# conix-center/pointcloud_stitching

Measured on AMD Instinct MI355X. Metric: Mpoints/s stitched (8x1280x720 streams: deproject+transform+RGB+pack), higher is better.
Workload: dtype f32

## Files before the change

pointcloud_stitching_amd/csrc/pcs_kernels.hip:

```cpp

#include "pcs_kernels_common.h"

#ifndef EMIT_WAVES
#define EMIT_WAVES 6
#endif

#ifndef PCS_SCALAR_FP64
#define PCS_SCALAR_FP64 0
#endif
#ifndef SCALAR_DENSE_WAVES
#define SCALAR_DENSE_WAVES 7
#endif
#ifndef SCALAR_EMIT_CUT_WAVES
#define SCALAR_EMIT_CUT_WAVES 5
#endif

namespace pcs {

namespace {

constexpr uint32_t kDenseStageBytes = kTilePoints * PCS_POINT_BYTES;
constexpr uint32_t kStageBytes      = kTilePoints * PCS_POINT_BYTES + 32;

__device__ __forceinline__ void stage_record(uint8_t* lds, uint32_t off, const Record& r)
// ... 73 lines not shown
#pragma unroll
            for (int k = 0; k < 8; k++) {
                const size_t i = (size_t)i0 + k;
                if (i < n) p[k] = PointIn{vertices[3 * i], vertices[3 * i + 1], vertices[3 * i + 2], texcoords[2 * i], texcoords[2 * i + 1]};
                else p[k] = PointIn{0, 0, 0, 0, 0};
            }
        }
    }
};

template <uint32_t THREADS = kBlockThreads>
__device__ __forceinline__ void store_staged(const uint8_t* lds, uint32_t head, uint32_t nbytes, uint8_t* g)
{
    uint8_t* g0 = g - head;
    const uint32_t end = head + nbytes;
    const uint32_t first_full = (head + 15u) >> 4;
    const uint32_t last_full = end >> 4;
    typedef uint32_t u32x4 __attribute__((ext_vector_type(4)));
    for (uint32_t j = first_full + threadIdx.x; j < last_full; j += THREADS)
        __builtin_nontemporal_store(reinterpret_cast<const u32x4*>(lds)[j], reinterpret_cast<u32x4*>(g0) + j);
    const uint32_t head_end = min(first_full << 4, end);
    for (uint32_t b = head + 2u * threadIdx.x; b < head_end; b += 2u * THREADS)
        *reinterpret_cast<uint16_t*>(g0 + b) = *reinterpret_cast<const uint16_t*>(lds + b);
    if (last_full >= first_full) {
        const uint32_t tail_begin = max(last_full << 4, head_end);
        for (uint32_t b = tail_begin + 2u * threadIdx.x; b < end; b += 2u * THREADS)
            *reinterpret_cast<uint16_t*>(g0 + b) = *reinterpret_cast<const uint16_t*>(lds + b);
    }
}

template <class Src, uint32_t THREADS = kBlockThreads, class Arith = SimdArith>
__device__ __forceinline__ void dense_tile(const StreamParams& P, const Src& src, const uint8_t* __restrict__ color,
                                           uint32_t tile0, uint32_t n, uint8_t* __restrict__ out_bytes,
                                           uint4* stage)
{
    const uint32_t i0 = tile0 + threadIdx.x * kPointsPerLane;
    PointIn p[8];
    src.load8(P, i0, n, p);

    uint32_t w[20];
    auto fill = [&](auto& cv) {
#pragma unroll
        for (int k = 0; k < 8; k += 2) {
            const Record a = make_record<Arith>(P, color, p[k], cv);
            const Record b = make_record<Arith>(P, color, p[k + 1], cv);
            uint32_t* o = w + (k >> 1) * 5;
            o[0] = a.xy;
            o[1] = a.zc;
            o[2] = perm(b.xy, a.b, kLoLo);
            o[3] = perm(b.zc, b.xy, kHiLo);
            o[4] = perm(b.b, b.zc, kHiLo);
        }
    };
    if (Src::Math::kCvtMode == 2) {
        FastCvt<false> fast;
        fill(fast);
        if (__builtin_expect(fast.redo(), 0)) { ExactCvt exact; fill(exact); }
    } else if (Src::Math::kCvtMode == 1) {
        FastCvt<true> fast;
        fill(fast);
        if (__builtin_expect(fast.redo(), 0)) { ExactCvt exact; fill(exact); }
    } else {
        ExactCvt exact;
        fill(exact);
    }
    uint4* mine = stage + threadIdx.x * 5;
#pragma unroll
    for (int k = 0; k < 5; k++) mine[k] = make_uint4(w[4 * k], w[4 * k + 1], w[4 * k + 2], w[4 * k + 3]);
    __syncthreads();

    const uint32_t pts = min(THREADS * kPointsPerLane, n - tile0);
    store_staged<THREADS>(reinterpret_cast<const uint8_t*>(stage), 0u, pts * PCS_POINT_BYTES,
                          out_bytes + (size_t)tile0 * PCS_POINT_BYTES);
}

constexpr uint32_t kWaveStageBytes = 64u * kPointsPerLane * PCS_POINT_BYTES;
constexpr uint32_t kWinPieces      = 3;
constexpr uint32_t kWinBytes       = kWinPieces * 64u * 16u;
constexpr uint32_t kWinZeroWord    = kWaveStageBytes - 16u;
static_assert(kWinBytes + 8u <= kWinZeroWord, "the windows, the dword read past their end and the zero word fit one wave's stage");

template <class T> using cptr = const __attribute__((address_space(4))) T*;

__device__ __forceinline__ void color_stretch(const StreamParams& P, const int32_t (&wp)[3], int32_t crow, int32_t c0, int32_t c1,
                                              uint32_t room, uint32_t& ws, uint32_t& len)
{
    const int32_t lo = min(max((c0 * wp[0] + wp[1]) >> 12, 0), P.cW - 1);
    const int32_t hi = min(max((c1 * wp[0] + wp[2]) >> 12, 0), P.cW - 1);
    const uint32_t row = (uint32_t)crow * (uint32_t)P.stride;
    ws = (row + (uint32_t)lo * (uint32_t)P.bpp) & ~15u;
    const uint32_t we = min((row + (uint32_t)hi * (uint32_t)P.bpp + 4u + 15u) & ~15u, P.color_bytes & ~15u);
    len = min(we > ws ? we - ws : 0u, room);
}

typedef uint32_t u32x4v __attribute__((ext_vector_type(4)));
__device__ __forceinline__ u32x4v load16_asm(const void* base, uint32_t off)
{
    u32x4v v;
    asm volatile("global_load_dwordx4 %0, %1, %2" : "=v"(v) : "v"(off), "s"(base));
    return v;
}
__device__ __forceinline__ uint32_t load4_asm(const void* base, uint32_t off)
{
    uint32_t v;
    asm volatile("global_load_dword %0, %1, %2" : "=v"(v) : "v"(off), "s"(base));
    return v;
}
__device__ __forceinline__ void window_piece(const uint8_t* color, uint32_t off, uint32_t lds)
{
    uint32_t keep;
    asm volatile("s_mov_b32 %0, m0\n\ts_mov_b32 m0, %3\n\ts_nop 0\n\tglobal_load_lds_dwordx4 %1, %2\n\ts_mov_b32 m0, %0"
                 : "=&s"(keep) : "v"(off), "s"(color), "s"(lds) : "memory");
}

template <class Mth>
__device__ __forceinline__ PointIn deproject_pixel_win(const StreamParams& P, uint32_t d, float mx, float my)
{
    const float z = __fmul_rn(P.depth_scale, (float)d);
    PointIn p;
    p.X = __fmul_rn(z, mx);
    p.Y = __fmul_rn(z, my);
    p.Z = z;
    const float P0 = __fadd_rn(p.X, P.t[0]);
    const float P2 = p.Z;
    float x, y_unused;
    Mth::div2(P0, P0, P2, x, y_unused);
    const float px = __fadd_rn(__fmul_rn(x, P.c_fx), P.c_ppx);
    p.u = Mth::div_const(px, P.c_w_f, P.c_rw);
    p.v = 0.0f;
    return p;
}

template <class Mth, uint32_t THREADS = kBlockThreads>
__device__ __forceinline__ void dense_tile_rowc(const StreamParams& P, const uint16_t* __restrict__ depth,
                                                const uint8_t* __restrict__ color, uint32_t tile0, uint32_t n,
                                                uint8_t* __restrict__ out_bytes, uint4* stage)
{
    static_assert(Mth::kRowConst && Mth::kCvtMode == 2, "the no-overflow row-constant policy");
    const uint32_t i0 = tile0 + threadIdx.x * kPointsPerLane;
    const uint32_t ic = min(i0, n - kPointsPerLane);
    const uint32_t r = P.w_magic ? (__umulhi(ic, P.w_magic) >> P.w_shift) : ic / (uint32_t)P.W;
    const uint32_t c0 = ic - r * (uint32_t)P.W;
    u32x4v dv = load16_asm(depth, ic * 2u);
    u32x4v ma = load16_asm(P.mx, c0 * 4u);
    u32x4v mb = load16_asm(P.mx, c0 * 4u + 16u);
    uint32_t myb = load4_asm(P.my, r * 4u);
    uint32_t crow = load4_asm(P.my, ((uint32_t)P.H + r) * 4u);

    const uint32_t wave = __builtin_amdgcn_readfirstlane(threadIdx.x >> 6);
    const uint32_t iw = tile0 + wave * 64u * kPointsPerLane;
    const uint32_t il = min(iw + 64u * kPointsPerLane, n) - 1u;
    const uint32_t ra = __builtin_amdgcn_readfirstlane(r), rb = __builtin_amdgcn_readlane(r, 63);
    const cptr<int32_t> tab = (cptr<int32_t>)(uintptr_t)(P.my + P.H);
    const int32_t wp[3] = {tab[P.H], tab[P.H + 1], tab[P.H + 2]};
    const uint32_t lrel = wave * kWaveStageBytes;
    uint32_t wsa = 0, lena = 0, wsb = 0, lenb = 0;
    if (iw < n) {
        color_stretch(P, wp, tab[ra], (int32_t)(iw - ra * (uint32_t)P.W), ra == rb ? (int32_t)(il - ra * (uint32_t)P.W) : P.W - 1,
                      kWinBytes, wsa, lena);
        if (rb != ra) color_stretch(P, wp, tab[rb], 0, (int32_t)(il - rb * (uint32_t)P.W), kWinBytes - lena, wsb, lenb);
    }
    const uint32_t lane = threadIdx.x & 63u;
    const uint32_t pieces = max((lena + lenb) >> 4, 1u), pa = lena >> 4;
    const uint32_t lds0 = (uint32_t)(uintptr_t)(__attribute__((address_space(3))) uint8_t*)stage + lrel;
#pragma unroll
    for (uint32_t k = 0; k < kWinPieces; k++) {
        const uint32_t j = min(k * 64u + lane, pieces - 1u);
        window_piece(color, j < pa ? wsa + 16u * j : wsb + 16u * (j - pa), lds0 + k * 1024u);
    }
    if (lane == 0) *reinterpret_cast<uint32_t*>(reinterpret_cast<uint8_t*>(stage) + lrel + kWinZeroWord) = *(cptr<uint32_t>)(uintptr_t)color;
    float M[12];
#pragma unroll
    for (int k = 0; k < 12; k++) M[k] = P.M[k];
    float c_wm1_f = P.c_wm1_f;
    uint32_t bpp = (uint32_t)P.bpp, stride = (uint32_t)P.stride;
    asm volatile("" : "+s"(M[0]), "+s"(M[1]), "+s"(M[2]), "+s"(M[3]), "+s"(M[4]), "+s"(M[5]), "+s"(M[6]), "+s"(M[7]), "+s"(M[8]),
                      "+s"(M[9]), "+s"(M[10]), "+s"(M[11]), "+s"(c_wm1_f), "+s"(bpp), "+s"(stride));
    static_assert(kWinPieces == 3, "the wait below leaves the window's requests in flight");
    asm volatile("s_waitcnt vmcnt(3)" : "+v"(dv), "+v"(ma), "+v"(mb), "+v"(myb), "+v"(crow));
    PointIn p[8];
    {
        const uint32_t dw[4] = {dv.x, dv.y, dv.z, dv.w};
        const uint32_t mxs[8] = {ma.x, ma.y, ma.z, ma.w, mb.x, mb.y, mb.z, mb.w};
#pragma unroll
        for (int k = 0; k < 8; k++) {
            const uint32_t d = (k & 1) ? (dw[k >> 1] >> 16) : (dw[k >> 1] & 0xFFFFu);
            p[k] = deproject_pixel_win<Mth>(P, d, __uint_as_float(mxs[k]), __uint_as_float(myb));
        }
    }
    FastCvt<false> cv;
    uint32_t xy[8], zz[8], ci[8];
    const uint32_t row_off = __umul24(crow, stride);
#pragma unroll
    for (int k = 0; k < 8; k++) {
        const float ax = world_mm(M + 0, p[k].X, p[k].Y, p[k].Z);
        const float ay = world_mm(M + 4, p[k].X, p[k].Y, p[k].Z);
        const float az = world_mm(M + 8, p[k].X, p[k].Y, p[k].Z);
        xy[k] = perm((uint32_t)cv.cvt(ay), (uint32_t)cv.cvt(ax), kLoLo);
        zz[k] = (uint32_t)cv.cvt(az);
        const int32_t xi = cv.pixel(__fmaf_rn(p[k].u, P.c_w_f, 0.5f), P.cW - 1, c_wm1_f);
        ci[k] = p[k].Z != 0.0f ? __umul24((uint32_t)xi, bpp) + row_off : 0u;
    }
    const bool in_a = r == ra;
    const uint32_t ws = in_a ? wsa : wsb, len = in_a ? lena : lenb;
    const uint32_t wn = len > 3u ? len - 3u : 0u;
    const uint32_t lb = lrel + (in_a ? 0u : lena), lz = lrel + kWinZeroWord;
    asm volatile("s_waitcnt vmcnt(0)" : "+v"(ci[0]), "+v"(ci[1]), "+v"(ci[2]), "+v"(ci[3]), "+v"(ci[4]), "+v"(ci[5]), "+v"(ci[6]),
                 "+v"(ci[7]) :: "memory");
    uint32_t wc[8];
    bool miss = false;
#pragma unroll
    for (int k = 0; k < 8; k++) {
        const uint32_t o = ci[k] - ws;
        const bool in = o < wn;
        const uint32_t* qa = reinterpret_cast<const uint32_t*>(reinterpret_cast<const uint8_t*>(stage) + (in ? (lb + o) & ~3u : lz));
        wc[k] = __builtin_amdgcn_alignbyte(qa[1], qa[0], ci[k]);
        miss |= !in && ci[k] != 0u;
    }
    if (__builtin_expect(miss, 0)) {
#pragma unroll
        for (int k = 0; k < 8; k++) {
            if (!(ci[k] - ws < wn) && ci[k] != 0u) {
                ExactCvt exact;
                uint32_t shift;
                const uint32_t off = exact.window(ci[k], P.color_bytes - 4u, shift);
                uint32_t g;
                __builtin_memcpy(&g, color + off, 4);
                wc[k] = g >> shift;
            }
        }
    }
    uint32_t w[20];
#pragma unroll
    for (int k = 0; k < 8; k += 2) {
        const Record a{xy[k], perm(wc[k], zz[k], kLoLo), __builtin_amdgcn_ubfe(wc[k], 16, 8)};
        const Record b{xy[k + 1], perm(wc[k + 1], zz[k + 1], kLoLo), __builtin_amdgcn_ubfe(wc[k + 1], 16, 8)};
        uint32_t* o = w + (k >> 1) * 5;
        o[0] = a.xy;
        o[1] = a.zc;
        o[2] = perm(b.xy, a.b, kLoLo);
        o[3] = perm(b.zc, b.xy, kHiLo);
        o[4] = perm(b.b, b.zc, kHiLo);
    }
    uint4* mine = stage + threadIdx.x * 5;
#pragma unroll
    for (int k = 0; k < 5; k++) mine[k] = make_uint4(w[4 * k], w[4 * k + 1], w[4 * k + 2], w[4 * k + 3]);
    __syncthreads();

    const uint32_t pts = min(THREADS * kPointsPerLane, n - tile0);
    store_staged<THREADS>(reinterpret_cast<const uint8_t*>(stage), 0u, pts * PCS_POINT_BYTES,
                          out_bytes + (size_t)tile0 * PCS_POINT_BYTES);
}

template <class Src, bool PRED, bool DS1, class Arith = SimdArith>
__device__ __forceinline__ void generic_tile(const StreamParams& P, const Src& src, const uint8_t* __restrict__ color,
                                             uint32_t tile0, uint32_t n, uint32_t flags, uint32_t ds,
                                             uint32_t g0, uint32_t out_first, uint8_t* __restrict__ payload_bytes,
                                             uint8_t* stage, uint32_t* wsum)
{
    if (DS1) ds = 1u;
    const uint32_t i0 = tile0 + threadIdx.x * kPointsPerLane;
    PointIn p[8];
    src.load8(P, i0, n, p);

    uint32_t keep, ex = 0;
    if (PRED) {
        keep = keep_mask8(p, i0, n, flags);
        uint32_t wave_total;
        ex = wave_exclusive_scan(__popc(keep), wave_total);
        if ((threadIdx.x & 63) == 63) wsum[threadIdx.x >> 6] = wave_total;
    } else {
        const uint32_t mine = (i0 < n) ? min(8u, n - i0) : 0u;
        keep = (1u << mine) - 1u;
    }

    Record rec[8];
    auto fill = [&](auto& cv) {
#pragma unroll
        for (int k = 0; k < 8; k++) rec[k] = make_record<Arith>(P, color, p[k], cv);
    };
    if (Src::Math::kCvtMode == 2) {
        FastCvt<false> fast;
        fill(fast);
        if (__builtin_expect(fast.redo(), 0)) { ExactCvt exact; fill(exact); }
    } else if (Src::Math::kCvtMode == 1) {
        FastCvt<true> fast;
        fill(fast);
        if (__builtin_expect(fast.redo(), 0)) { ExactCvt exact; fill(exact); }
    } else {
        ExactCvt exact;
        fill(exact);
    }

    uint32_t lane_first, tile_kept;
    if (PRED) {
        __syncthreads();
        const int wave = threadIdx.x >> 6;
        uint32_t before = 0;
        for (int w = 0; w < wave; w++) before += wsum[w];
        tile_kept = wsum[0] + wsum[1] + wsum[2] + wsum[3];
        lane_first = before + ex;
    } else {
        const uint32_t pts = min(kTilePoints, n - tile0);
        lane_first = min(threadIdx.x * kPointsPerLane, pts);
        tile_kept = pts;
    }

    const uint32_t q_lo = out_first + (DS1 ? g0 : (g0 + ds - 1) / ds);
    const uint32_t q_hi = out_first + (DS1 ? g0 + tile_kept : (g0 + tile_kept + ds - 1) / ds);
    uint8_t* gdst = payload_bytes + (size_t)q_lo * PCS_POINT_BYTES;
    const uint32_t head = (uint32_t)((uintptr_t)gdst & 15u);

    uint32_t g = g0 + lane_first;
// ... 76 lines not shown
    const uint32_t n = P.n_points;
    const uint32_t tile0 = t * kTilePoints;
    const uint32_t i0 = tile0 + threadIdx.x * kPointsPerLane;
    const uint8_t* __restrict__ color = fp.color[s];

    DepthSource<true, true, Mth> src{fp.depth[s]};
    PointIn p[8];
    src.load8(P, i0, n, p);
    const uint32_t keep = keep_mask8(p, i0, n, a.flags);

    uint32_t wave_total;
    const uint32_t ex = wave_exclusive_scan(__popc(keep), wave_total);
    const int wave = threadIdx.x >> 6, lane = threadIdx.x & 63;
    if (lane == 63) wsum[wave] = wave_total;
    __syncthreads();
    uint32_t before = 0;
    for (int w = 0; w < wave; w++) before += wsum[w];
    const uint32_t tile_kept = wsum[0] + wsum[1] + wsum[2] + wsum[3];
    const uint32_t lane_first = before + ex;

    if (threadIdx.x == 0)
        __hip_atomic_store(a.desc + gtile, desc_pack(a.gen, kDescReady, tile_kept), __ATOMIC_RELAXED,
                           __HIP_MEMORY_SCOPE_AGENT);

    Record rec[8];
    auto fill = [&](auto& cv) {
#pragma unroll
        for (int k = 0; k < 8; k++) rec[k] = make_record(P, color, p[k], cv);
    };
    if (Mth::kCvtMode == 2) {
        FastCvt<false> fast;
        fill(fast);
        if (__builtin_expect(fast.redo(), 0)) { ExactCvt exact; fill(exact); }
    } else if (Mth::kCvtMode == 1) {
        FastCvt<true> fast;
        fill(fast);
        if (__builtin_expect(fast.redo(), 0)) { ExactCvt exact; fill(exact); }
    } else {
        ExactCvt exact;
        fill(exact);
    }

    uint32_t own = 0, tot = 0;
    const uint32_t first = gtile - t;
    for (uint32_t j = first + threadIdx.x; j < gtile; j += kBlockThreads) own += desc_wait(a.desc + j, a.gen, a.error);
    if ((int)threadIdx.x < s) tot = desc_wait(a.stream_desc + stream0 + threadIdx.x, a.gen, a.error);
    const uint32_t tot_lane = tot;
    own = wave_sum(own);
    tot = wave_sum(tot);
    if (lane == 0) { psum[wave] = own; psum[4 + wave] = tot; }
    __syncthreads();
    const uint32_t own_excl = psum[0] + psum[1] + psum[2] + psum[3];
    const uint32_t chain = a.chain_in ? *a.chain_in : 0u;
    const uint32_t q_lo = chain + psum[4] + psum[5] + psum[6] + psum[7] + own_excl;
    if (threadIdx.x == 0 && t == tiles_s - 1) {
        __hip_atomic_store(a.stream_desc + stream0 + s, desc_pack(a.gen, kDescReady, own_excl + tile_kept), __ATOMIC_RELAXED,
                           __HIP_MEMORY_SCOPE_AGENT);
        a.stream_end[stream0 + s] = q_lo + tile_kept;
    }
    if (a.counts && s == n_launch - 1 && t == tiles_s - 1) {
        if ((int)threadIdx.x < s) a.counts[stream0 + threadIdx.x] = (int32_t)tot_lane;
        if (threadIdx.x == 0) {
            a.counts[stream0 + s] = (int32_t)(own_excl + tile_kept);
            if (a.last_launch) a.counts[a.n_total] = (int32_t)(q_lo + tile_kept);
        }
    }

    uint8_t* gdst = payload_bytes + (size_t)q_lo * PCS_POINT_BYTES;
    const uint32_t head = (uint32_t)((uintptr_t)gdst & 15u);
    uint32_t rank = lane_first;
#pragma unroll
    for (int k = 0; k < 8; k++) {
        if ((keep >> k) & 1u) {
            stage_record(stage, head + rank * PCS_POINT_BYTES, rec[k]);
            rank++;
        }
    }
    __syncthreads();
    store_staged(stage, head, tile_kept * PCS_POINT_BYTES, gdst);
}



template <bool DDIST, bool CDIST, class Mth, uint32_t THREADS = kBlockThreads>
__global__ __launch_bounds__(THREADS, 7)
void pcs_fused_dense_kernel(const StreamParams* __restrict__ params, int stream0, FramePtrs fp,
                            uint8_t* __restrict__ payload_bytes)
{
    __shared__ uint4 stage[THREADS * kPointsPerLane * PCS_POINT_BYTES / 16];
    const int s = blockIdx.y;
    const StreamParams& P = params[stream0 + s];
    request_constants(P, fp.depth[s], fp.color[s], payload_bytes);
    const uint32_t n = P.n_points;
    const uint32_t tile0 = blockIdx.x * (THREADS * kPointsPerLane);
    if (tile0 >= n) return;
    if constexpr (Mth::kRowConst) {
        dense_tile_rowc<Mth, THREADS>(P, fp.depth[s], fp.color[s], tile0, n, payload_bytes + (size_t)P.out_base * PCS_POINT_BYTES, stage);
    } else {
        DepthSource<DDIST, CDIST, Mth> src{fp.depth[s]};
        dense_tile<DepthSource<DDIST, CDIST, Mth>, THREADS>(P, src, fp.color[s], tile0, n, payload_bytes + (size_t)P.out_base * PCS_POINT_BYTES, stage);
    }
}

template <bool DDIST, bool CDIST, class Mth>
__global__ __launch_bounds__(kBlockThreads, 7)
void pcs_fused_dense_batch_kernel(const StreamParams* __restrict__ params, BatchPtrs bp)
{
    __shared__ uint4 stage[kDenseStageBytes / 16];
    const int s = blockIdx.y;
    const StreamParams& P = params[s];
    const int e = blockIdx.z * gridDim.y + s;
    request_constants(P, bp.depth[e], bp.color[e], bp.payload[blockIdx.z]);
    const uint32_t n = P.n_points;
    const uint32_t tile0 = blockIdx.x * kTilePoints;
    if (tile0 >= n) return;
    if constexpr (Mth::kRowConst) {
        dense_tile_rowc<Mth>(P, bp.depth[e], bp.color[e], tile0, n, bp.payload[blockIdx.z] + (size_t)P.out_base * PCS_POINT_BYTES, stage);
    } else {
        DepthSource<DDIST, CDIST, Mth> src{bp.depth[e]};
        dense_tile(P, src, bp.color[e], tile0, n, bp.payload[blockIdx.z] + (size_t)P.out_base * PCS_POINT_BYTES, stage);
    }
}

constexpr int kCountTiles = 2;
template <bool DDIST, bool CDIST>
__device__ __forceinline__ void count_tiles(const StreamParams& P, const uint16_t* __restrict__ dp, uint32_t flags,
                                            uint32_t* __restrict__ tile_counts, uint32_t (*wsum)[4])
{
    const uint32_t n = P.n_points;
    const uint32_t tile_first = blockIdx.x * kCountTiles;
    if (tile_first * kTilePoints >= n) return;
    uint32_t c[kCountTiles];
    const bool cut = (flags & PCS_FLAG_CUTOFF) != 0;
    if (P.z_zero_iff_d_zero && (!cut || P.cut_dmax != 0u)) {
        const uint32_t dmax = cut ? P.cut_dmax : 0xFFFFu;
        uint4 dv[kCountTiles];
        const bool aligned = ((uintptr_t)dp & 15) == 0 && n >= 8;
        if (aligned) {
#pragma unroll
            for (int q = 0; q < kCountTiles; q++) {
                const uint32_t i0 = (tile_first + q) * kTilePoints + threadIdx.x * kPointsPerLane;
                dv[q] = *reinterpret_cast<const uint4*>(dp + ((i0 + 8 <= n) ? i0 : 0u));
            }
        } else {
#pragma unroll
            for (int q = 0; q < kCountTiles; q++) dv[q] = make_uint4(0, 0, 0, 0);
        }
#pragma unroll
        for (int q = 0; q < kCountTiles; q++) {
            const uint32_t i0 = (tile_first + q) * kTilePoints + threadIdx.x * kPointsPerLane;
            uint32_t dw[4] = {dv[q].x, dv[q].y, dv[q].z, dv[q].w};
            if (!(aligned && i0 + 8 <= n)) {
                dw[0] = dw[1] = dw[2] = dw[3] = 0u;
                for (uint32_t k = 0; k < 8 && i0 + k < n; k++) dw[k >> 1] |= (uint32_t)dp[i0 + k] << ((k & 1u) * 16u);
            }
            uint32_t rng = 0, nz = 0;
#pragma unroll
            for (int k = 0; k < 8; k++) {
                const uint32_t d = (k & 1) ? (dw[k >> 1] >> 16) : (dw[k >> 1] & 0xFFFFu);
                nz  |= (uint32_t)(d != 0u) << k;
                rng |= (uint32_t)(d != 0u && d <= dmax) << k;
            }
            c[q] = __popc(keep_from_bits(rng, nz, i0, n, flags));
        }
    } else {
        DepthSource<DDIST, CDIST> src{dp};
#pragma unroll
        for (int q = 0; q < kCountTiles; q++) {
            const uint32_t i0 = (tile_first + q) * kTilePoints + threadIdx.x * kPointsPerLane;
            PointIn p[8];
            src.load8(P, i0, n, p);
            c[q] = __popc(keep_mask8(p, i0, n, flags));
        }
    }
#pragma unroll
    for (int q = 0; q < kCountTiles; q++) {
        const uint32_t w = wave_sum(c[q]);
        if ((threadIdx.x & 63) == 0) wsum[q][threadIdx.x >> 6] = w;
    }
    __syncthreads();
    if (threadIdx.x < kCountTiles && (tile_first + threadIdx.x) * kTilePoints < n)
        tile_counts[P.tile_base + tile_first + threadIdx.x] =
            wsum[threadIdx.x][0] + wsum[threadIdx.x][1] + wsum[threadIdx.x][2] + wsum[threadIdx.x][3];
}

template <bool DDIST, bool CDIST>
__global__ __launch_bounds__(kBlockThreads)
void pcs_fused_count_kernel(const StreamParams* __restrict__ params, int stream0, FramePtrs fp, uint32_t flags,
                            uint32_t* __restrict__ tile_counts)
{
    __shared__ uint32_t wsum[kCountTiles][4];
    const int s = blockIdx.y;
    count_tiles<DDIST, CDIST>(params[stream0 + s], fp.depth[s], flags, tile_counts, wsum);
}

template <bool DDIST, bool CDIST>
__global__ __launch_bounds__(kBlockThreads)
void pcs_fused_count_batch_kernel(const StreamParams* __restrict__ params, BatchPtrs bp, uint32_t flags,
                                  uint32_t* __restrict__ tile_counts, uint32_t total_tiles)
{
    __shared__ uint32_t wsum[kCountTiles][4];
    const int s = blockIdx.y;
    count_tiles<DDIST, CDIST>(params[s], bp.depth[blockIdx.z * gridDim.y + s], flags,
                              tile_counts + (size_t)blockIdx.z * total_tiles, wsum);
// ... 539 lines not shown
        if (noovf)      { if (ident) L(false, false, CertIdentNoOvf); else L(false, false, CertNoOvf); }
        else if (ident) { if (any_cdist) L(false, true, CertMath<true>); else L(false, false, CertMath<true>); }
        else            { if (any_cdist) L(false, true, CertMath<false>); else L(false, false, CertMath<false>); }
    } else {
        if (any_ddist) { if (any_cdist) L(true, true, IeeeMath); else L(true, false, IeeeMath); }
        else           { if (any_cdist) L(false, true, IeeeMath); else L(false, false, IeeeMath); }
    }
#undef L
    return hipGetLastError();
}

hipError_t launch_fused_count(const StreamParams* d_params, int stream0, int n_launch, uint32_t max_points,
                              uint32_t flags, const FramePtrs& fp, uint32_t* d_tile_counts, hipStream_t st)
{
    if (n_launch <= 0 || max_points == 0) return hipSuccess;
    const uint32_t tiles = (max_points + kTilePoints - 1) / kTilePoints;
    const dim3 grid((tiles + kCountTiles - 1) / kCountTiles, (unsigned)n_launch, 1);
    hipLaunchKernelGGL((pcs_fused_count_kernel<true, false>), grid, dim3(kBlockThreads), 0, st,
                       d_params, stream0, fp, flags, d_tile_counts);
    return hipGetLastError();
}

hipError_t launch_scan(const StreamParams* d_params, int n_streams, int downsample,
                       const uint32_t* d_tile_counts, uint32_t* d_tile_prefix, uint32_t* d_stream_kept,
                       int32_t* d_counts, uint32_t* d_arrive, hipStream_t st)
{
    hipLaunchKernelGGL(pcs_scan_kernel, dim3((unsigned)n_streams), dim3(1024), 0, st, d_params, 0, n_streams, 0u,
                       (uint32_t)downsample, d_tile_counts, d_tile_prefix, d_stream_kept, d_counts, d_arrive);
    return hipGetLastError();
}

hipError_t launch_fused_emit(const StreamParams* d_params, int stream0, int n_launch, uint32_t max_points,
                             uint32_t flags, int downsample, MathSel math, const FramePtrs& fp,
                             const uint32_t* d_tile_prefix, const uint32_t* d_stream_kept,
                             int16_t* d_payload, int32_t* d_total_out, int n_total_streams, hipStream_t st)
{
    if (n_launch <= 0 || max_points == 0) return hipSuccess;
    const dim3 grid = tile_grid(max_points, n_launch);
    const bool pred = (flags & (PCS_FLAG_CUTOFF | PCS_FLAG_DROP_INVALID)) != 0;
    const bool ds1 = downsample == 1;
    uint8_t* out = reinterpret_cast<uint8_t*>(d_payload);
#define L(PR, D1, M) hipLaunchKernelGGL((pcs_fused_emit_kernel<PR, D1, M>), grid, dim3(kBlockThreads), 0, st, d_params, \
                                        stream0, fp, flags, (uint32_t)downsample, d_tile_prefix, d_stream_kept, out, \
                                        d_total_out, n_total_streams)
#define LM(M) do { if (pred) { if (ds1) L(true, true, M); else L(true, false, M); } \
                   else      { if (ds1) L(false, true, M); else L(false, false, M); } } while (0)
    const bool ident = (math == MathSel::CertIdentR || math == MathSel::CertIdentRNoOvf);
    if (math == MathSel::Ieee) LM(IeeeMath); else if (ident) LM(CertMath<true>); else LM(CertMath<false>);
#undef LM
#undef L
    return hipGetLastError();
}

hipError_t launch_fused_compact(const StreamParams* d_params, int stream0, int n_launch, uint32_t launch_tiles,
                                MathSel math, const FramePtrs& fp, const CompactLaunch& cl, int16_t* d_payload,
                                hipStream_t st)
{
    if (n_launch <= 0 || launch_tiles == 0) return hipSuccess;
    CompactArgs a;
    a.ticket = cl.d_ticket; a.ticket_base = cl.ticket_base; a.desc = cl.d_desc; a.stream_desc = cl.d_stream_desc;
    a.stream_end = cl.d_stream_end;
    a.chain_in = cl.d_chain_in; a.error = cl.d_error; a.gen = cl.gen & 0x3FFFFFFFu; a.flags = cl.flags;
    a.counts = cl.d_counts; a.n_total = cl.n_total; a.last_launch = cl.last_launch;
    uint8_t* out = reinterpret_cast<uint8_t*>(d_payload);
    if (math != MathSel::Ieee)
        hipLaunchKernelGGL((pcs_fused_compact_kernel<CertMath<false>>), dim3(launch_tiles), dim3(kBlockThreads), 0, st,
                           d_params, stream0, n_launch, fp, a, out);
    else
        hipLaunchKernelGGL((pcs_fused_compact_kernel<IeeeMath>), dim3(launch_tiles), dim3(kBlockThreads), 0, st,
                           d_params, stream0, n_launch, fp, a, out);
    return hipGetLastError();
}

hipError_t launch_fused_dense_batch(const StreamParams* d_params, int n_streams, int n_sets, uint32_t max_points,
                                    bool any_ddist, bool any_cdist, MathSel math, const BatchPtrs& bp, hipStream_t st)
{
    if (n_streams <= 0 || n_sets <= 0 || max_points == 0) return hipSuccess;
    if (n_streams * n_sets > kBatchEntries || n_sets > kBatchSets) return hipErrorInvalidValue;
    const dim3 grid((max_points + kTilePoints - 1) / kTilePoints, (unsigned)n_streams, (unsigned)n_sets);
#define L(DD, CD, M) hipLaunchKernelGGL((pcs_fused_dense_batch_kernel<DD, CD, M>), grid, dim3(kBlockThreads), 0, st, d_params, bp)
    if (math == MathSel::CertRowConstNoOvf) {
        bool aligned = !any_ddist && !any_cdist;
        for (int k = 0; k < n_streams * n_sets; k++) aligned &= ((((uintptr_t)bp.color[k]) | ((uintptr_t)bp.depth[k])) & 15u) == 0;
        if (aligned) { L(false, false, CertRowConstNoOvf); return hipGetLastError(); }
        math = MathSel::CertIdentRNoOvf;
    }
    if (math != MathSel::Ieee && !any_ddist) {
        const bool ident = (math == MathSel::CertIdentR || math == MathSel::CertIdentRNoOvf);
        const bool noovf = (math == MathSel::CertNoOvf || math == MathSel::CertIdentRNoOvf) && !any_cdist;
        if (noovf)      { if (ident) L(false, false, CertIdentNoOvf); else L(false, false, CertNoOvf); }
        else if (ident) { if (any_cdist) L(false, true, CertMath<true>); else L(false, false, CertMath<true>); }
        else            { if (any_cdist) L(false, true, CertMath<false>); else L(false, false, CertMath<false>); }
    } else {
        if (any_ddist) { if (any_cdist) L(true, true, IeeeMath); else L(true, false, IeeeMath); }
        else           { if (any_cdist) L(false, true, IeeeMath); else L(false, false, IeeeMath); }
    }
#undef L
    return hipGetLastError();
}

hipError_t launch_compact_batch(const StreamParams* d_params, int n_streams, int n_sets, uint32_t max_points,
                                uint32_t total_tiles, uint32_t flags, MathSel math, const BatchPtrs& bp,
                                const BatchCounts& bc, uint32_t* d_tile_counts, uint32_t* d_tile_prefix,
                                uint32_t* d_stream_kept, hipStream_t st)
{
    if (n_streams <= 0 || n_sets <= 0 || max_points == 0) return hipSuccess;
    if (n_streams * n_sets > kBatchEntries || n_sets > kBatchSets) return hipErrorInvalidValue;
    const uint32_t tiles = (max_points + kTilePoints - 1) / kTilePoints;
    hipLaunchKernelGGL((pcs_fused_count_batch_kernel<true, false>),
                       dim3((tiles + kCountTiles - 1) / kCountTiles, (unsigned)n_streams, (unsigned)n_sets),
                       dim3(kBlockThreads), 0, st, d_params, bp, flags, d_tile_counts, total_tiles);
    hipLaunchKernelGGL(pcs_scan_batch_kernel, dim3((unsigned)n_streams, (unsigned)n_sets), dim3(1024), 0, st, d_params,
                       d_tile_counts, d_tile_prefix, d_stream_kept, total_tiles, bc);
    const dim3 grid(tiles, (unsigned)n_streams, (unsigned)n_sets);
#define L(M) hipLaunchKernelGGL((pcs_fused_emit_batch_kernel<M>), grid, dim3(kBlockThreads), 0, st, d_params, bp, flags, \
                                d_tile_prefix, d_stream_kept, total_tiles, bc)
    const bool ident = (math == MathSel::CertIdentR || math == MathSel::CertIdentRNoOvf);
    if (math == MathSel::Ieee) L(IeeeMath); else if (ident) L(CertMath<true>); else L(CertMath<false>);
#undef L
    return hipGetLastError();
}

hipError_t launch_pack_batch(const StreamParams* d_params, const PackBatch& pb, int n, uint32_t max_points, bool aligned,
                             hipStream_t st)
{
    if (n <= 0 || max_points == 0) return hipSuccess;
    if (n > kPackBatch) return hipErrorInvalidValue;
    const dim3 grid = tile_grid(max_points, n);
    if (aligned) hipLaunchKernelGGL((pcs_pack_batch_kernel<true>), grid, dim3(kBlockThreads), 0, st, d_params, pb);
    else         hipLaunchKernelGGL((pcs_pack_batch_kernel<false>), grid, dim3(kBlockThreads), 0, st, d_params, pb);
    return hipGetLastError();
}

hipError_t launch_certify_color_row(const StreamParams* d_params, int stream, int rows, int32_t* d_crow, unsigned long long* d_bad, hipStream_t st)
{
    if (rows <= 0) return hipSuccess;
    hipLaunchKernelGGL(pcs_certify_color_row_kernel, dim3((unsigned)rows), dim3(256), 0, st, d_params, stream, d_crow, d_bad);
    return hipGetLastError();
}

hipError_t launch_verify_div_const(float c, float rc, int32_t dim, unsigned long long* d_bad, hipStream_t st)
{
    hipLaunchKernelGGL(pcs_verify_div_const_kernel, dim3(8192), dim3(256), 0, st, c, rc, dim, d_bad);
    return hipGetLastError();
}

hipError_t launch_pack_dense(const StreamParams* d_params, int stream, const VertexPtrs& vp,
                             int16_t* d_out, hipStream_t st)
{
    if (vp.n_points == 0) return hipSuccess;
    if (small_launch(vp.n_points, 1))
        hipLaunchKernelGGL((pcs_pack_dense_kernel<kSmallThreads>), dim3((vp.n_points + kSmallTilePoints - 1) / kSmallTilePoints),
                           dim3(kSmallThreads), 0, st, d_params, stream, vp, reinterpret_cast<uint8_t*>(d_out));
    else
        hipLaunchKernelGGL((pcs_pack_dense_kernel<kBlockThreads>), tile_grid(vp.n_points, 1), dim3(kBlockThreads), 0, st,
                           d_params, stream, vp, reinterpret_cast<uint8_t*>(d_out));
    return hipGetLastError();
}

hipError_t launch_pack_count(const StreamParams* d_params, int stream, const VertexPtrs& vp, uint32_t flags,
                             uint32_t* d_tile_counts, hipStream_t st)
{
    if (vp.n_points == 0) return hipSuccess;
    hipLaunchKernelGGL(pcs_pack_count_kernel, tile_grid(vp.n_points, 1), dim3(kBlockThreads), 0, st,
                       d_params, stream, vp, flags, d_tile_counts);
    return hipGetLastError();
}
// ... 103 lines not shown
```

Measured before the change: 341,100.

## Batch scalar parameter loads into explicit SMEM bursts in row-constant dense tile

Replaces the row-constant dense tile's scattered StreamParams and kernarg reads with a few hand-written s_load bursts. One burst fetches the header words, the LUT and frame pointers, and a second fetches the matrix, the intrinsics, the color-window table entries and the zero word, each followed by a single lgkmcnt wait. This cuts the chain of dependent scalar-load latencies before the first vector loads issue. The rare miss-path color gathers are also made branch-free, issuing all eight loads before one wait. It adds a dedicated batch kernel signature and hard-coded struct offsets guarded by static_asserts, which makes the code fragile to layout changes.

```diff
diff --git a/pointcloud_stitching_amd/csrc/pcs_kernels.hip b/pointcloud_stitching_amd/csrc/pcs_kernels.hip
--- a/pointcloud_stitching_amd/csrc/pcs_kernels.hip
+++ b/pointcloud_stitching_amd/csrc/pcs_kernels.hip
@@ -179,7 +179,14 @@
 
 template <class T> using cptr = const __attribute__((address_space(4))) T*;
 
-__device__ __forceinline__ void color_stretch(const StreamParams& P, const int32_t (&wp)[3], int32_t crow, int32_t c0, int32_t c1,
+struct RowcParams {
+    float    M[12];
+    float    t0, depth_scale, c_fx, c_ppx, c_w_f, c_wm1_f, c_rw;
+    int32_t  W, H, cW, bpp, stride;
+    uint32_t color_bytes, n_points, out_base, w_magic, w_shift;
+};
+
+__device__ __forceinline__ void color_stretch(const RowcParams& P, const int32_t (&wp)[3], int32_t crow, int32_t c0, int32_t c1,
                                               uint32_t room, uint32_t& ws, uint32_t& len)
 {
     const int32_t lo = min(max((c0 * wp[0] + wp[1]) >> 12, 0), P.cW - 1);
@@ -211,14 +218,14 @@
 }
 
 template <class Mth>
-__device__ __forceinline__ PointIn deproject_pixel_win(const StreamParams& P, uint32_t d, float mx, float my)
+__device__ __forceinline__ PointIn deproject_pixel_win(const RowcParams& P, uint32_t d, float mx, float my)
 {
     const float z = __fmul_rn(P.depth_scale, (float)d);
     PointIn p;
     p.X = __fmul_rn(z, mx);
     p.Y = __fmul_rn(z, my);
     p.Z = z;
-    const float P0 = __fadd_rn(p.X, P.t[0]);
+    const float P0 = __fadd_rn(p.X, P.t0);
     const float P2 = p.Z;
     float x, y_unused;
     Mth::div2(P0, P0, P2, x, y_unused);
@@ -228,34 +235,100 @@
     return p;
 }
 
+typedef uint32_t u32x8s __attribute__((ext_vector_type(8)));
+typedef uint32_t u32x16s __attribute__((ext_vector_type(16)));
+template <class T> using karg = const __attribute__((address_space(4))) T*;
+
 template <class Mth, uint32_t THREADS = kBlockThreads>
-__device__ __forceinline__ void dense_tile_rowc(const StreamParams& P, const uint16_t* __restrict__ depth,
-                                                const uint8_t* __restrict__ color, uint32_t tile0, uint32_t n,
-                                                uint8_t* __restrict__ out_bytes, uint4* stage)
+__device__ __forceinline__ void dense_tile_rowc(const StreamParams* Pp, karg<const uint16_t*> depth_arg, karg<const uint8_t*> color_arg,
+                                                karg<uint8_t*> payload_arg, uint4* stage)
 {
     static_assert(Mth::kRowConst && Mth::kCvtMode == 2, "the no-overflow row-constant policy");
+    static_assert(offsetof(StreamParams, ck) + 4 * 4 == 0xc0 && offsetof(StreamParams, W) == 0xc4 && offsetof(StreamParams, H) == 0xc8 &&
+                  offsetof(StreamParams, cW) == 0xcc && offsetof(StreamParams, bpp) == 0xd4 && offsetof(StreamParams, stride) == 0xd8 &&
+                  offsetof(StreamParams, color_bytes) == 0xdc && offsetof(StreamParams, n_points) == 0xe0 &&
+                  offsetof(StreamParams, out_base) == 0xec && offsetof(StreamParams, w_magic) == 0xf4 &&
+                  offsetof(StreamParams, w_shift) == 0xf8 && offsetof(StreamParams, M) == 0, "the head's sixteen words from 0xc0; M at 0");
+    RowcParams P;
+    const float* lut_x;
+    const float* lut_y;
+    const uint16_t* depth;
+    const uint8_t* color;
+    __attribute__((address_space(1))) uint8_t* payload_bytes;
+    {
+        u32x16s g;
+        asm volatile("s_load_dwordx16 %0, %6, 0xc0\n\t"
+                     "s_load_dwordx2 %1, %6, %10\n\t"
+                     "s_load_dwordx2 %2, %6, %11\n\t"
+                     "s_load_dwordx2 %3, %7, 0x0\n\t"
+                     "s_load_dwordx2 %4, %8, 0x0\n\t"
+                     "s_load_dwordx2 %5, %9, 0x0\n\t"
+                     "s_waitcnt lgkmcnt(0)"
+                     : "=&s"(g), "=&s"(lut_x), "=&s"(lut_y), "=&s"(depth), "=&s"(color), "=&s"(payload_bytes)
+                     : "s"(Pp), "s"(depth_arg), "s"(color_arg), "s"(payload_arg),
+                       "n"(offsetof(StreamParams, mx)), "n"(offsetof(StreamParams, my)));
+        P.W = (int32_t)g[1]; P.H = (int32_t)g[2]; P.cW = (int32_t)g[3]; P.bpp = (int32_t)g[5]; P.stride = (int32_t)g[6];
+        P.color_bytes = g[7]; P.n_points = g[8]; P.out_base = g[11]; P.w_magic = g[13]; P.w_shift = g[14];
+    }
+    const uint32_t n = P.n_points;
+    const uint32_t tile0 = blockIdx.x * (THREADS * kPointsPerLane);
+    if (tile0 >= n) return;
+    uint8_t* out_bytes = (uint8_t*)payload_bytes + (size_t)P.out_base * PCS_POINT_BYTES;
     const uint32_t i0 = tile0 + threadIdx.x * kPointsPerLane;
     const uint32_t ic = min(i0, n - kPointsPerLane);
     const uint32_t r = P.w_magic ? (__umulhi(ic, P.w_magic) >> P.w_shift) : ic / (uint32_t)P.W;
     const uint32_t c0 = ic - r * (uint32_t)P.W;
     u32x4v dv = load16_asm(depth, ic * 2u);
-    u32x4v ma = load16_asm(P.mx, c0 * 4u);
-    u32x4v mb = load16_asm(P.mx, c0 * 4u + 16u);
-    uint32_t myb = load4_asm(P.my, r * 4u);
-    uint32_t crow = load4_asm(P.my, ((uint32_t)P.H + r) * 4u);
+    u32x4v ma = load16_asm(lut_x, c0 * 4u);
+    u32x4v mb = load16_asm(lut_x, c0 * 4u + 16u);
+    uint32_t myb = load4_asm(lut_y, r * 4u);
+    uint32_t crow = load4_asm(lut_y, ((uint32_t)P.H + r) * 4u);
 
     const uint32_t wave = __builtin_amdgcn_readfirstlane(threadIdx.x >> 6);
     const uint32_t iw = tile0 + wave * 64u * kPointsPerLane;
     const uint32_t il = min(iw + 64u * kPointsPerLane, n) - 1u;
     const uint32_t ra = __builtin_amdgcn_readfirstlane(r), rb = __builtin_amdgcn_readlane(r, 63);
-    const cptr<int32_t> tab = (cptr<int32_t>)(uintptr_t)(P.my + P.H);
-    const int32_t wp[3] = {tab[P.H], tab[P.H + 1], tab[P.H + 2]};
+    const cptr<int32_t> tab = (cptr<int32_t>)(uintptr_t)(lut_y + P.H);
+    int32_t wp[3], crow_a, crow_b;
+    uint32_t word0;
+    {
+        u32x8s m0;
+        u32x4v m8;
+        uint64_t w01;
+        asm volatile("s_load_dwordx8 %0, %14, 0x0\n\t"
+                     "s_load_dwordx4 %1, %14, 0x20\n\t"
+                     "s_load_dword %2, %14, %19\n\t"
+                     "s_load_dword %3, %14, %20\n\t"
+                     "s_load_dword %4, %14, %21\n\t"
+                     "s_load_dword %5, %14, %22\n\t"
+                     "s_load_dword %6, %14, %23\n\t"
+                     "s_load_dword %7, %14, %24\n\t"
+                     "s_load_dword %8, %14, %25\n\t"
+                     "s_load_dwordx2 %9, %15, 0x0\n\t"
+                     "s_load_dword %10, %15, 0x8\n\t"
+                     "s_load_dword %11, %16, 0x0\n\t"
+                     "s_load_dword %12, %17, 0x0\n\t"
+                     "s_load_dword %13, %18, 0x0\n\t"
+                     "s_waitcnt lgkmcnt(0)"
+                     : "=&s"(m0), "=&s"(m8), "=&s"(P.t0), "=&s"(P.depth_scale), "=&s"(P.c_fx), "=&s"(P.c_ppx), "=&s"(P.c_w_f),
+                       "=&s"(P.c_wm1_f), "=&s"(P.c_rw), "=&s"(w01), "=&s"(wp[2]), "=&s"(crow_a), "=&s"(crow_b), "=&s"(word0)
+                     : "s"(Pp), "s"(tab + P.H), "s"(tab + ra), "s"(tab + rb), "s"(color),
+                       "n"(offsetof(StreamParams, t)), "n"(offsetof(StreamParams, depth_scale)), "n"(offsetof(StreamParams, c_fx)),
+                       "n"(offsetof(StreamParams, c_ppx)), "n"(offsetof(StreamParams, c_w_f)), "n"(offsetof(StreamParams, c_wm1_f)),
+                       "n"(offsetof(StreamParams, c_rw)));
+#pragma unroll
+        for (int k = 0; k < 8; k++) P.M[k] = __uint_as_float(m0[k]);
+#pragma unroll
+        for (int k = 0; k < 4; k++) P.M[8 + k] = __uint_as_float(m8[k]);
+        wp[0] = (int32_t)(uint32_t)w01;
+        wp[1] = (int32_t)(uint32_t)(w01 >> 32);
+    }
     const uint32_t lrel = wave * kWaveStageBytes;
     uint32_t wsa = 0, lena = 0, wsb = 0, lenb = 0;
     if (iw < n) {
-        color_stretch(P, wp, tab[ra], (int32_t)(iw - ra * (uint32_t)P.W), ra == rb ? (int32_t)(il - ra * (uint32_t)P.W) : P.W - 1,
+        color_stretch(P, wp, crow_a, (int32_t)(iw - ra * (uint32_t)P.W), ra == rb ? (int32_t)(il - ra * (uint32_t)P.W) : P.W - 1,
                       kWinBytes, wsa, lena);
-        if (rb != ra) color_stretch(P, wp, tab[rb], 0, (int32_t)(il - rb * (uint32_t)P.W), kWinBytes - lena, wsb, lenb);
+        if (rb != ra) color_stretch(P, wp, crow_b, 0, (int32_t)(il - rb * (uint32_t)P.W), kWinBytes - lena, wsb, lenb);
     }
     const uint32_t lane = threadIdx.x & 63u;
     const uint32_t pieces = max((lena + lenb) >> 4, 1u), pa = lena >> 4;
@@ -265,14 +338,10 @@
         const uint32_t j = min(k * 64u + lane, pieces - 1u);
         window_piece(color, j < pa ? wsa + 16u * j : wsb + 16u * (j - pa), lds0 + k * 1024u);
     }
-    if (lane == 0) *reinterpret_cast<uint32_t*>(reinterpret_cast<uint8_t*>(stage) + lrel + kWinZeroWord) = *(cptr<uint32_t>)(uintptr_t)color;
-    float M[12];
-#pragma unroll
-    for (int k = 0; k < 12; k++) M[k] = P.M[k];
-    float c_wm1_f = P.c_wm1_f;
-    uint32_t bpp = (uint32_t)P.bpp, stride = (uint32_t)P.stride;
-    asm volatile("" : "+s"(M[0]), "+s"(M[1]), "+s"(M[2]), "+s"(M[3]), "+s"(M[4]), "+s"(M[5]), "+s"(M[6]), "+s"(M[7]), "+s"(M[8]),
-                      "+s"(M[9]), "+s"(M[10]), "+s"(M[11]), "+s"(c_wm1_f), "+s"(bpp), "+s"(stride));
+    if (lane == 0) *reinterpret_cast<uint32_t*>(reinterpret_cast<uint8_t*>(stage) + lrel + kWinZeroWord) = word0;
+    const float* M = P.M;
+    const float c_wm1_f = P.c_wm1_f;
+    const uint32_t bpp = (uint32_t)P.bpp, stride = (uint32_t)P.stride;
     static_assert(kWinPieces == 3, "the wait below leaves the window's requests in flight");
     asm volatile("s_waitcnt vmcnt(3)" : "+v"(dv), "+v"(ma), "+v"(mb), "+v"(myb), "+v"(crow));
     PointIn p[8];
@@ -315,17 +384,17 @@
         miss |= !in && ci[k] != 0u;
     }
     if (__builtin_expect(miss, 0)) {
+        uint32_t g[8], shift[8];
 #pragma unroll
         for (int k = 0; k < 8; k++) {
-            if (!(ci[k] - ws < wn) && ci[k] != 0u) {
-                ExactCvt exact;
-                uint32_t shift;
-                const uint32_t off = exact.window(ci[k], P.color_bytes - 4u, shift);
-                uint32_t g;
-                __builtin_memcpy(&g, color + off, 4);
-                wc[k] = g >> shift;
-            }
+            ExactCvt exact;
+            const bool gather = !(ci[k] - ws < wn) && ci[k] != 0u;
+            g[k] = load4_asm(color, exact.window(gather ? ci[k] : 0u, P.color_bytes - 4u, shift[k]));
         }
+        asm volatile("s_waitcnt vmcnt(0)" : "+v"(g[0]), "+v"(g[1]), "+v"(g[2]), "+v"(g[3]), "+v"(g[4]), "+v"(g[5]), "+v"(g[6]), "+v"(g[7]));
+#pragma unroll
+        for (int k = 0; k < 8; k++)
+            if (!(ci[k] - ws < wn) && ci[k] != 0u) wc[k] = g[k] >> shift[k];
     }
     uint32_t w[20];
 #pragma unroll
@@ -568,6 +637,9 @@
 
 
 
+struct DenseKernArgs { const StreamParams* params; int stream0; FramePtrs fp; uint8_t* payload_bytes; };
+struct BatchKernArgs { const StreamParams* params; int n_streams; BatchPtrs bp; };
+
 template <bool DDIST, bool CDIST, class Mth, uint32_t THREADS = kBlockThreads>
 __global__ __launch_bounds__(THREADS, 7)
 void pcs_fused_dense_kernel(const StreamParams* __restrict__ params, int stream0, FramePtrs fp,
@@ -575,14 +647,18 @@
 {
     __shared__ uint4 stage[THREADS * kPointsPerLane * PCS_POINT_BYTES / 16];
     const int s = blockIdx.y;
-    const StreamParams& P = params[stream0 + s];
-    request_constants(P, fp.depth[s], fp.color[s], payload_bytes);
-    const uint32_t n = P.n_points;
-    const uint32_t tile0 = blockIdx.x * (THREADS * kPointsPerLane);
-    if (tile0 >= n) return;
     if constexpr (Mth::kRowConst) {
-        dense_tile_rowc<Mth, THREADS>(P, fp.depth[s], fp.color[s], tile0, n, payload_bytes + (size_t)P.out_base * PCS_POINT_BYTES, stage);
+        const auto args = (karg<uint8_t>)__builtin_amdgcn_kernarg_segment_ptr();
+        dense_tile_rowc<Mth, THREADS>(params + (stream0 + s),
+                                      (karg<const uint16_t*>)(args + offsetof(DenseKernArgs, fp) + offsetof(FramePtrs, depth)) + s,
+                                      (karg<const uint8_t*>)(args + offsetof(DenseKernArgs, fp) + offsetof(FramePtrs, color)) + s,
+                                      (karg<uint8_t*>)(args + offsetof(DenseKernArgs, payload_bytes)), stage);
     } else {
+        const StreamParams& P = params[stream0 + s];
+        request_constants(P, fp.depth[s], fp.color[s], payload_bytes);
+        const uint32_t n = P.n_points;
+        const uint32_t tile0 = blockIdx.x * (THREADS * kPointsPerLane);
+        if (tile0 >= n) return;
         DepthSource<DDIST, CDIST, Mth> src{fp.depth[s]};
         dense_tile<DepthSource<DDIST, CDIST, Mth>, THREADS>(P, src, fp.color[s], tile0, n, payload_bytes + (size_t)P.out_base * PCS_POINT_BYTES, stage);
     }
@@ -592,6 +668,7 @@
 __global__ __launch_bounds__(kBlockThreads, 7)
 void pcs_fused_dense_batch_kernel(const StreamParams* __restrict__ params, BatchPtrs bp)
 {
+    static_assert(!Mth::kRowConst, "the row-constant tile has its own K-set kernel (below)");
     __shared__ uint4 stage[kDenseStageBytes / 16];
     const int s = blockIdx.y;
     const StreamParams& P = params[s];
@@ -600,12 +677,22 @@
     const uint32_t n = P.n_points;
     const uint32_t tile0 = blockIdx.x * kTilePoints;
     if (tile0 >= n) return;
-    if constexpr (Mth::kRowConst) {
-        dense_tile_rowc<Mth>(P, bp.depth[e], bp.color[e], tile0, n, bp.payload[blockIdx.z] + (size_t)P.out_base * PCS_POINT_BYTES, stage);
-    } else {
-        DepthSource<DDIST, CDIST, Mth> src{bp.depth[e]};
-        dense_tile(P, src, bp.color[e], tile0, n, bp.payload[blockIdx.z] + (size_t)P.out_base * PCS_POINT_BYTES, stage);
-    }
+    DepthSource<DDIST, CDIST, Mth> src{bp.depth[e]};
+    dense_tile(P, src, bp.color[e], tile0, n, bp.payload[blockIdx.z] + (size_t)P.out_base * PCS_POINT_BYTES, stage);
+}
+
+template <class Mth>
+__global__ __launch_bounds__(kBlockThreads, 7)
+void pcs_fused_dense_batch_kernel(const StreamParams* __restrict__ params, int n_streams, BatchPtrs bp)
+{
+    static_assert(Mth::kRowConst, "the row-constant tile's K-set kernel");
+    __shared__ uint4 stage[kDenseStageBytes / 16];
+    const int s = blockIdx.y;
+    const int e = blockIdx.z * n_streams + s;
+    const auto args = (karg<uint8_t>)__builtin_amdgcn_kernarg_segment_ptr();
+    dense_tile_rowc<Mth>(params + s, (karg<const uint16_t*>)(args + offsetof(BatchKernArgs, bp) + offsetof(BatchPtrs, depth)) + e,
+                         (karg<const uint8_t*>)(args + offsetof(BatchKernArgs, bp) + offsetof(BatchPtrs, color)) + e,
+                         (karg<uint8_t*>)(args + offsetof(BatchKernArgs, bp) + offsetof(BatchPtrs, payload)) + blockIdx.z, stage);
 }
 
 constexpr int kCountTiles = 2;
@@ -1311,7 +1398,10 @@
     if (math == MathSel::CertRowConstNoOvf) {
         bool aligned = !any_ddist && !any_cdist;
         for (int k = 0; k < n_streams * n_sets; k++) aligned &= ((((uintptr_t)bp.color[k]) | ((uintptr_t)bp.depth[k])) & 15u) == 0;
-        if (aligned) { L(false, false, CertRowConstNoOvf); return hipGetLastError(); }
+        if (aligned) {
+            hipLaunchKernelGGL((pcs_fused_dense_batch_kernel<CertRowConstNoOvf>), grid, dim3(kBlockThreads), 0, st, d_params, n_streams, bp);
+            return hipGetLastError();
+        }
         math = MathSel::CertIdentRNoOvf;
     }
     if (math != MathSel::Ieee && !any_ddist) {
```

Result: no change. 343,000 (median of 6 runs) (+0.6%).
